# tqch/ddpm-torch

Measured on AMD Instinct MI355X. Metric: training imgs/s/GPU + 1000-step DDPM samples/s, CIFAR-10 UNet @1/2/4/8 MI355X, higher is better.
Workload: dtype bf16

## Files before the change

ddpm-torch_amd/csrc/attention.hip:

```cpp
#include "common.h"
#include "attention_common.h"
#include <string.h>

namespace {

constexpr int RB = 128;
constexpr int NT = 512;

struct AttnArgs {
    const bf16_t *q, *k, *v;  long long qkv_ld;
    const bf16_t *o, *d_o;    long long o_ld, do_ld;
    bf16_t *out;              long long out_ld;
    bf16_t *dq, *dk, *dv;     long long dqkv_ld;
    float *lse, *dvec;
    int B, L, C, Lpad;
    float scale;
};

__device__ __forceinline__ int tile_addr(int row, int col, int pitch_b, int km) {
    return row * pitch_b + ((((col >> 3) ^ (row & km))) << 4) + (col & 7) * 2;
}

template <int NJ>
struct P1 {
    f32x16 acc[2][NJ];
    __device__ __forceinline__ void zero() {
#pragma unroll
        for (int i = 0; i < 2; ++i)
#pragma unroll
            for (int j = 0; j < NJ; ++j) acc[i][j] = (f32x16)(0.f);
    }
};

__device__ __forceinline__ void wait_vm_rt(int n) {
    switch (n) {
    case 0: asm volatile("s_waitcnt vmcnt(0)" ::: "memory"); break;
    case 1: asm volatile("s_waitcnt vmcnt(1)" ::: "memory"); break;
    case 2: asm volatile("s_waitcnt vmcnt(2)" ::: "memory"); break;
    case 3: asm volatile("s_waitcnt vmcnt(3)" ::: "memory"); break;
    case 4: asm volatile("s_waitcnt vmcnt(4)" ::: "memory"); break;
    case 5: asm volatile("s_waitcnt vmcnt(5)" ::: "memory"); break;
    case 6: asm volatile("s_waitcnt vmcnt(6)" ::: "memory"); break;
    case 7: asm volatile("s_waitcnt vmcnt(7)" ::: "memory"); break;
    default: asm volatile("s_waitcnt vmcnt(8)" ::: "memory"); break;
    }
}

#ifdef ATTN_TIMING
__device__ unsigned long long* g_attn_timing = nullptr;
#define ATTN_STAMP(slot) do { if (g_attn_timing && threadIdx.x == 0) g_attn_timing[(blockIdx.y * gridDim.x + blockIdx.x) * 8 + (slot)] = wall_clock64(); } while (0)
#else
#define ATTN_STAMP(slot)
#endif

constexpr int P1_RING = 3, P2_RING = 5;
constexpr int P2_SLOT = 2 * NT * 16;
__device__ __host__ __forceinline__ int p1_slot_bytes(int Lpad) { return RB * 128 + ((Lpad + 63) / 64) * 8192; }
__device__ __host__ __forceinline__ int p2_rows(int C) { return C > 256 ? 16 : (C > 128 ? 32 : 64); }

template <int NJ, bool PIPE = true>
__device__ __forceinline__ void product_nt(P1<NJ>& t, const Opnd& X, int r0, const Opnd& Y, int Lpad, int C, char* lds, int tid) {
    const int lane = tid & 63, wr = (tid >> 8) & 1, wc = (tid >> 6) & 3;
    const int wave = __builtin_amdgcn_readfirstlane(tid >> 6);
    const int nyi = (Lpad + 63) / 64;
    const int xs_bytes = RB * 128, slot_bytes = p1_slot_bytes(Lpad), per = 2 + nyi;
    const unsigned lds0 = lds_addr(lds);
    const int nchunks = (C + 63) / 64;
    unsigned xo[2], yo[4]; int xc[2], yc[4];
#pragma unroll
    for (int i = 0; i < 2; ++i) {
        const int v = tid + NT * i, row = v >> 3;
        xc[i] = ((v & 7) ^ ((row >> 1) & 7)) * 8;
        xo[i] = (unsigned)(((long long)(r0 + row) * X.ld + xc[i]) * 2);
    }
#pragma unroll
    for (int i = 0; i < 4; ++i) {
        const int v = tid + NT * i, row = v >> 3;
        yc[i] = ((v & 7) ^ ((row >> 1) & 7)) * 8;
        yo[i] = row < Lpad ? (unsigned)(((long long)row * Y.ld + yc[i]) * 2) : BUF_OOB;
    }
    auto issue = [&](int ch) {
        char* slot = lds + (ch % P1_RING) * slot_bytes;
        const int c0 = ch * 64;
#pragma unroll
        for (int i = 0; i < 2; ++i) {
            unsigned o = c0 + xc[i] < C ? xo[i] + (unsigned)(c0 * 2) : BUF_OOB;
            asm volatile("" : "+v"(o));
            LDS_DMA16(X.rsrc, slot + (i * NT + wave * 64) * 16, o, 0);
        }
#pragma unroll
        for (int i = 0; i < 4; ++i) {
            if (i < nyi) {
                unsigned o = (yo[i] != BUF_OOB && c0 + yc[i] < C) ? yo[i] + (unsigned)(c0 * 2) : BUF_OOB;
                asm volatile("" : "+v"(o));
                LDS_DMA16(Y.rsrc, slot + xs_bytes + (i * NT + wave * 64) * 16, o, 0);
            }
        }
    };
    issue(0);
    if (nchunks > 1) issue(1);
    const int sw = (lane >> 5) ^ ((lane >> 1) & 7);
    const unsigned arow = (unsigned)((wr * 64 + (lane & 31)) * 128), brow = (unsigned)(xs_bytes + (wc * 32 + (lane & 31)) * 128);
    bool jok[NJ];
#pragma unroll
    for (int j = 0; j < NJ; ++j) jok[j] = (wc + 4 * j) * 32 < Lpad;
#ifdef ATTN_TIMING
    unsigned long long tq[5] = {0, 0, 0, 0, 0};
#define P1_T(k) do { if (ch == 1) tq[k] = clock64(); } while (0)
#else
#define P1_T(k)
#endif
    for (int ch = 0; ch < nchunks; ++ch) {
        P1_T(0);
        wait_vm_rt(ch + 1 < nchunks ? per : 0);
        P1_T(1);
        __builtin_amdgcn_s_barrier();
        P1_T(2);
        if (ch + 2 < nchunks) issue(ch + 2);
        P1_T(3);
        const unsigned cur = lds0 + (unsigned)((ch % P1_RING) * slot_bytes);
        constexpr int NS = PIPE ? 2 : 1;
        u32x4 fa[NS][2], fb[NS][NJ];
        auto rd = [&](int kc, int set) {
            const unsigned ko = (unsigned)(((2 * kc) ^ sw) << 4);
#pragma unroll
            for (int i = 0; i < 2; ++i) fa[set][i] = lds_rd16(cur + arow + (unsigned)(i * 32 * 128) + ko);
#pragma unroll
            for (int j = 0; j < NJ; ++j) fb[set][j] = lds_rd16(cur + (jok[j] ? brow + (unsigned)(j * 128 * 128) : (unsigned)xs_bytes) + ko);
        };
        rd(0, 0);
#pragma unroll
        for (int kc = 0; kc < 4; ++kc) {
            constexpr int cs = NS == 2 ? 1 : 0;
            if (NS == 1) { if (kc > 0) rd(kc, 0); lds_wait_n<0>(); }
            else if (kc < 3) { rd(kc + 1, (kc + 1) & 1); lds_wait_n<2 + NJ>(); } else lds_wait_n<0>();
#pragma unroll
            for (int i = 0; i < 2; ++i)
#pragma unroll
                for (int j = 0; j < NJ; ++j)
                    if (jok[j]) t.acc[i][j] = __builtin_amdgcn_mfma_f32_32x32x16_bf16(as_frag(fa[kc & cs][i]), as_frag(fb[kc & cs][j]), t.acc[i][j], 0, 0, 0);
            __builtin_amdgcn_sched_barrier(0);
        }
        P1_T(4);
    }
#ifdef ATTN_TIMING
    if (g_attn_timing && threadIdx.x == 0 && tq[4])
        g_attn_timing[(blockIdx.y * gridDim.x + blockIdx.x) * 8 + 7] = ((tq[1] - tq[0]) & 0xffff) | (((tq[2] - tq[1]) & 0xffff) << 16) | (((tq[3] - tq[2]) & 0xffff) << 32) | (((tq[4] - tq[3]) & 0xffff) << 48);
#endif
#undef P1_T
    __syncthreads();
}

template <int NJ2>
__device__ __forceinline__ void product_nn(f32x16 (&z)[2][NJ2], const char* tile, int pitch_b, int km, const Opnd& Y, int L, int Lpad, int C,
                                           char* ring, int tid) {
    const int lane = tid & 63, wr = (tid >> 8) & 1, wc = (tid >> 6) & 3;
    const int wave = __builtin_amdgcn_readfirstlane(tid >> 6);
    const int KR = p2_rows(C);
    const int row_b = C * 2, cpr = C >> 3;
    const int nvec = KR * cpr;
    const int skey = C % 128 == 0 ? 2 : 0;
#pragma unroll
    for (int i = 0; i < 2; ++i)
#pragma unroll
        for (int j = 0; j < NJ2; ++j) z[i][j] = (f32x16)(0.f);
    const int nchunks = (Lpad + KR - 1) / KR;
    int vkr[2]; unsigned vo[2];
#pragma unroll
    for (int i = 0; i < 2; ++i) {
        const int v = tid + NT * i;
        const int kr = v / cpr, pc = v - kr * cpr;
        const int lc = skey ? (pc ^ ((kr & 3) << 2)) : pc;
        vkr[i] = v < nvec ? kr : (1 << 20);
        vo[i] = (unsigned)(((long long)kr * Y.ld + lc * 8) * 2);
    }
    const unsigned kstep = (unsigned)((long long)KR * Y.ld * 2);
    auto issue = [&](int ch) {
        char* slot = ring + (ch % P2_RING) * P2_SLOT;
#pragma unroll
        for (int i = 0; i < 2; ++i) {
            unsigned o = ch * KR + vkr[i] < L ? vo[i] + (unsigned)ch * kstep : BUF_OOB;
            asm volatile("" : "+v"(o));
            LDS_DMA16(Y.rsrc, slot + (i * NT + wave * 64) * 16, o, 0);
        }
    };
    for (int c = 0; c < P2_RING - 1 && c < nchunks; ++c) issue(c);
    const int i16 = lane & 15;
    const unsigned tile0 = lds_addr(tile), ring0 = lds_addr(ring);
    bool jok[NJ2];
#pragma unroll
    for (int j = 0; j < NJ2; ++j) jok[j] = (wc + 4 * j) * 32 < C;
    for (int ch = 0; ch < nchunks; ++ch) {
        const int ahead = min(ch + P2_RING - 2, nchunks - 1) - ch;
        wait_vm_rt(2 * ahead);
        __builtin_amdgcn_s_barrier();
        if (ch + P2_RING - 1 < nchunks) issue(ch + P2_RING - 1);
        const unsigned cur = ring0 + (unsigned)((ch % P2_RING) * P2_SLOT);
        constexpr int NS = NJ2 <= 2 ? 2 : 1;
        u32x4 fa[NS][2]; uint2 fb[NS][NJ2][2];
        const int nks = min(KR / 16, (Lpad - ch * KR + 15) / 16);
        auto rd = [&](int ks, int set) {
            const int kg = ch * KR + ks * 16;
#pragma unroll
            for (int i = 0; i < 2; ++i) {
                const int row = wr * 64 + i * 32 + (lane & 31);
                fa[set][i] = lds_rd16(tile0 + (unsigned)(row * pitch_b + ((((kg >> 3) + (lane >> 5)) ^ (row & km)) << 4)));
            }
#pragma unroll
            for (int j = 0; j < NJ2; ++j) {
                const int ct = jok[j] ? wc + 4 * j : wc;
                const int mcol = ct * 32 + ((lane >> 4) & 1) * 16 + (i16 & 3) * 4;
                const int krow = ks * 16 + (lane >> 5) * 8 + (i16 >> 2);
                const int pch = skey ? ((mcol >> 3) ^ ((krow & 3) << 2)) : (mcol >> 3);
                const unsigned p = cur + (unsigned)(krow * row_b + pch * 16 + (mcol & 7) * 2);
                fb[set][j][0] = lds_rd_tr(p); fb[set][j][1] = lds_rd_tr(p + (unsigned)(4 * row_b));
            }
        };
        rd(0, 0);
        for (int ks = 0; ks < nks; ks += 2) {
#pragma unroll
            for (int h = 0; h < 2; ++h) {
                if (ks + h >= nks) break;
                constexpr int cs = NS == 2 ? 1 : 0;
                const int cur_set = h & cs;
                if (NS == 1) { if (ks + h > 0) rd(ks + h, 0); lds_wait_n<0>(); }
                else if (ks + h + 1 < nks) { rd(ks + h + 1, (h + 1) & 1); lds_wait_n<2 + 2 * NJ2>(); } else lds_wait_n<0>();
#pragma unroll
                for (int j = 0; j < NJ2; ++j) {
                    if (!jok[j]) continue;
                    u32x4 b4; b4.x = fb[cur_set][j][0].x; b4.y = fb[cur_set][j][0].y; b4.z = fb[cur_set][j][1].x; b4.w = fb[cur_set][j][1].y;
#pragma unroll
                    for (int i = 0; i < 2; ++i) z[i][j] = __builtin_amdgcn_mfma_f32_32x32x16_bf16(as_frag(fa[cur_set][i]), as_frag(b4), z[i][j], 0, 0, 0);
                }
                __builtin_amdgcn_sched_barrier(0);
            }
        }
    }
    __syncthreads();
}

template <int CNT, int OFF, typename Op>
__device__ __forceinline__ float half_reduce(const float (&v)[CNT], int lane, Op&& op) {
    if constexpr (CNT == 1) return v[0];
    else {
        const bool bit = (lane & OFF) != 0;
        float o[CNT / 2];
#pragma unroll
        for (int k = 0; k < CNT / 2; ++k) {
            const float send = bit ? v[k] : v[k + CNT / 2], keep = bit ? v[k + CNT / 2] : v[k];
            o[k] = op(keep, __shfl_xor(send, OFF, 64));
        }
        return half_reduce<CNT / 2, OFF / 2>(o, lane, op);
    }
}

__device__ __forceinline__ int acc_row(int r, int lane) { return (r & 3) + 8 * (r >> 2) + 4 * (lane >> 5); }

template <int NJ, typename F>
__device__ __forceinline__ void write_tile(const P1<NJ>& t, char* tile, int pitch_b, int km, int Lpad, int tid, F&& f) {
    const int lane = tid & 63, wave = tid >> 6, wr = wave >> 2, wc = wave & 3;
#pragma unroll
    for (int i = 0; i < 2; ++i)
#pragma unroll
        for (int j = 0; j < NJ; ++j) {
            const int ct = wc + 4 * j;
            if (ct * 32 >= Lpad) continue;
#pragma unroll
            for (int r = 0; r < 16; ++r) {
                const int row = wr * 64 + i * 32 + acc_row(r, lane), col = ct * 32 + (lane & 31);
                *reinterpret_cast<bf16_t*>(tile + tile_addr(row, col, pitch_b, km)) = f2bf(f(t.acc[i][j][r], i, j, r, row, col));
            }
        }
}

template <int NJ2>
__device__ __forceinline__ void store_rows(const f32x16 (&z)[2][NJ2], bf16_t* out, long long ld, int r0, int L, int C, int tid) {
    const int lane = tid & 63, wave = tid >> 6, wr = wave >> 2, wc = wave & 3;
#pragma unroll
    for (int i = 0; i < 2; ++i)
#pragma unroll
        for (int j = 0; j < NJ2; ++j) {
            const int ct = wc + 4 * j;
            if (ct * 32 >= C) continue;
#pragma unroll
            for (int r = 0; r < 16; ++r) {
                const int row = r0 + wr * 64 + i * 32 + acc_row(r, lane);
                if (row < L) out[(long long)row * ld + ct * 32 + (lane & 31)] = f2bf(z[i][j][r]);
            }
        }
}

__device__ __forceinline__ void attn_block(int B, int& b, int& r0) {
    const int gx = gridDim.x;
    if (gx > 1 && (B & 7) == 0) {
        const int L = blockIdx.y * gx + blockIdx.x, k = L >> 3;
        r0 = (k % gx) * RB;
        b = (k / gx) * 8 + (L & 7);
    } else { b = blockIdx.y; r0 = blockIdx.x * RB; }
}

struct Lds {
    char* tile; char* stage; float* red;
    int pitch_b, km;
};
__device__ __forceinline__ Lds carve(char* smem, int Lpad) {
    Lds l;
    l.pitch_b = Lpad * 2;
    const int nch = Lpad >> 3;
    int span = 4;
    while (span < 16 && nch % (span * 2) == 0) span *= 2;
    l.km = span - 1;
    l.tile = smem;
    l.stage = smem + RB * l.pitch_b;
    l.red = nullptr;
    return l;
}

template <int NJ1, int NJ2>
__global__ __launch_bounds__(NT, 2)
void attn_fwd_lse_kernel(AttnArgs a) {
    extern __shared__ __attribute__((aligned(16))) char smem[];
    const int tid = threadIdx.x, lane = tid & 63, wave = tid >> 6, wr = wave >> 2, wc = wave & 3;
    int b, r0;
    attn_block(a.B, b, r0);
    Lds l = carve(smem, a.Lpad);
    const Opnd Q = make_opnd(a.q + (long long)b * a.L * a.qkv_ld, a.qkv_ld, a.L, a.C);
    const Opnd K = make_opnd(a.k + (long long)b * a.L * a.qkv_ld, a.qkv_ld, a.L, a.C);
    const Opnd V = make_opnd(a.v + (long long)b * a.L * a.qkv_ld, a.qkv_ld, a.L, a.C);
    ATTN_STAMP(0);
    P1<NJ1> s;
    s.zero();
    product_nt<NJ1, (NJ2 <= 2)>(s, Q, r0, K, a.Lpad, a.C, smem, tid);
    ATTN_STAMP(1);
    float* red = reinterpret_cast<float*>(l.stage);
    const int kk = lane & 31, myrow = wr * 64 + (kk >> 4) * 32 + acc_row(kk & 15, lane);
    float vals[32];
#pragma unroll
    for (int i = 0; i < 2; ++i)
#pragma unroll
        for (int r = 0; r < 16; ++r) {
            float m = -3.0e38f;
#pragma unroll
            for (int j = 0; j < NJ1; ++j) {
                const int col = (wc + 4 * j) * 32 + (lane & 31);
                const float v = col < a.L ? s.acc[i][j][r] * a.scale : -3.0e38f;
                s.acc[i][j][r] = v;
                m = fmaxf(m, v);
            }
            vals[i * 16 + r] = m;
        }
    red[wc * RB + myrow] = half_reduce<32, 16>(vals, lane, [](float x, float y) { return fmaxf(x, y); });
    __syncthreads();
#pragma unroll
    for (int i = 0; i < 2; ++i)
#pragma unroll
        for (int r = 0; r < 16; ++r) {
            const int row = wr * 64 + i * 32 + acc_row(r, lane);
            const float m = fmaxf(fmaxf(red[row], red[RB + row]), fmaxf(red[2 * RB + row], red[3 * RB + row]));
            float sum = 0.f;
#pragma unroll
            for (int j = 0; j < NJ1; ++j) {
                const int col = (wc + 4 * j) * 32 + (lane & 31);
                const float e = col < a.L ? __expf(s.acc[i][j][r] - m) : 0.f;
                s.acc[i][j][r] = e;
                sum += e;
            }
            vals[i * 16 + r] = sum;
        }
    float* rsum = red + 4 * RB;
    rsum[wc * RB + myrow] = half_reduce<32, 16>(vals, lane, [](float x, float y) { return x + y; });
    __syncthreads();
    float rinv[2][16];
#pragma unroll
    for (int i = 0; i < 2; ++i)
#pragma unroll
        for (int r = 0; r < 16; ++r) {
            const int row = wr * 64 + i * 32 + acc_row(r, lane);
            const float tot = (rsum[row] + rsum[RB + row]) + (rsum[2 * RB + row] + rsum[3 * RB + row]);
            rinv[i][r] = __builtin_amdgcn_rcpf(tot);
        }
    if (a.lse && tid < RB && r0 + tid < a.L) {
        const float m = fmaxf(fmaxf(red[tid], red[RB + tid]), fmaxf(red[2 * RB + tid], red[3 * RB + tid]));
        const float tot = (rsum[tid] + rsum[RB + tid]) + (rsum[2 * RB + tid] + rsum[3 * RB + tid]);
        a.lse[(long long)b * a.L + r0 + tid] = m + __logf(tot);
    }
    __syncthreads();
    ATTN_STAMP(2);
    write_tile<NJ1>(s, l.tile, l.pitch_b, l.km, a.Lpad, tid, [&](float e, int i, int, int r, int, int) { return e * rinv[i][r]; });
    __syncthreads();
    ATTN_STAMP(3);
    f32x16 z[2][NJ2];
    product_nn<NJ2>(z, l.tile, l.pitch_b, l.km, V, a.L, a.Lpad, a.C, l.stage, tid);
    ATTN_STAMP(4);
    store_rows<NJ2>(z, a.out + (long long)b * a.L * a.out_ld, a.out_ld, r0, a.L, a.C, tid);
    ATTN_STAMP(5);
#ifdef ATTN_TIMING
    asm volatile("s_waitcnt vmcnt(0)" ::: "memory");
#endif
    ATTN_STAMP(6);
}

template <int NJ1, int NJ2>
__global__ __launch_bounds__(NT, 2)
void attn_bwd_dq_kernel(AttnArgs a) {
    extern __shared__ __attribute__((aligned(16))) char smem[];
    const int tid = threadIdx.x, lane = tid & 63, wave = tid >> 6, wr = wave >> 2, wc = wave & 3;
    int b, r0;
    attn_block(a.B, b, r0);
    Lds l = carve(smem, a.Lpad);
    const Opnd Q = make_opnd(a.q + (long long)b * a.L * a.qkv_ld, a.qkv_ld, a.L, a.C);
    const Opnd K = make_opnd(a.k + (long long)b * a.L * a.qkv_ld, a.qkv_ld, a.L, a.C);
    const Opnd V = make_opnd(a.v + (long long)b * a.L * a.qkv_ld, a.qkv_ld, a.L, a.C);
    const Opnd dO = make_opnd(a.d_o + (long long)b * a.L * a.do_ld, a.do_ld, a.L, a.C);
    float* dloc = reinterpret_cast<float*>(l.tile);
    {
        const int row = tid >> 2, part = tid & 3, q = r0 + row;
        float acc = 0.f;
        if (q < a.L) {
            const bf16_t* po = a.o + ((long long)b * a.L + q) * a.o_ld;
            const bf16_t* pd = a.d_o + ((long long)b * a.L + q) * a.do_ld;
            for (int c = part * 8; c < a.C; c += 32) {
                float fo[8], fd[8];
                Elem<bf16_t>::unpack(ldg16(po + c), fo); Elem<bf16_t>::unpack(ldg16(pd + c), fd);
#pragma unroll
                for (int e = 0; e < 8; ++e) acc += fo[e] * fd[e];
            }
        }
        acc += __shfl_xor(acc, 1, 64); acc += __shfl_xor(acc, 2, 64);
        if (part == 0) { dloc[row] = acc; if (q < a.L) a.dvec[(long long)b * a.L + q] = acc; }
    }
    __syncthreads();
    float drow[2][16], lrow[2][16];
#pragma unroll
    for (int i = 0; i < 2; ++i)
#pragma unroll
        for (int r = 0; r < 16; ++r) {
            const int row = wr * 64 + i * 32 + acc_row(r, lane), q = r0 + row;
            drow[i][r] = dloc[row];
            lrow[i][r] = q < a.L ? a.lse[(long long)b * a.L + q] : 0.f;
        }
    __syncthreads();
    P1<NJ1> p;
    p.zero();
    product_nt<NJ1, (NJ2 <= 2)>(p, Q, r0, K, a.Lpad, a.C, smem, tid);
#pragma unroll
    for (int i = 0; i < 2; ++i)
#pragma unroll
        for (int j = 0; j < NJ1; ++j)
#pragma unroll
            for (int r = 0; r < 16; ++r) {
                const int col = (wc + 4 * j) * 32 + (lane & 31);
                p.acc[i][j][r] = col < a.L ? __expf(p.acc[i][j][r] * a.scale - lrow[i][r]) : 0.f;
            }
    P1<NJ1> dp;
    dp.zero();
    product_nt<NJ1, (NJ2 <= 2)>(dp, dO, r0, V, a.Lpad, a.C, smem, tid);
    write_tile<NJ1>(dp, l.tile, l.pitch_b, l.km, a.Lpad, tid,
                    [&](float v, int i, int j, int r, int, int) { return p.acc[i][j][r] * (v - drow[i][r]) * a.scale; });
    __syncthreads();
    f32x16 z[2][NJ2];
    product_nn<NJ2>(z, l.tile, l.pitch_b, l.km, K, a.L, a.Lpad, a.C, l.stage, tid);
    store_rows<NJ2>(z, a.dq + (long long)b * a.L * a.dqkv_ld, a.dqkv_ld, r0, a.L, a.C, tid);
}

template <int NJ1, int NJ2>
__global__ __launch_bounds__(NT, 2)
void attn_bwd_dkv_kernel(AttnArgs a) {
    extern __shared__ __attribute__((aligned(16))) char smem[];
    const int tid = threadIdx.x, lane = tid & 63, wave = tid >> 6, wc = wave & 3;
    int b, r0;
    attn_block(a.B, b, r0);
    Lds l = carve(smem, a.Lpad);
    const Opnd Q = make_opnd(a.q + (long long)b * a.L * a.qkv_ld, a.qkv_ld, a.L, a.C);
    const Opnd K = make_opnd(a.k + (long long)b * a.L * a.qkv_ld, a.qkv_ld, a.L, a.C);
    const Opnd V = make_opnd(a.v + (long long)b * a.L * a.qkv_ld, a.qkv_ld, a.L, a.C);
    const Opnd dO = make_opnd(a.d_o + (long long)b * a.L * a.do_ld, a.do_ld, a.L, a.C);
    float lcol[NJ1], dcol[NJ1];
#pragma unroll
    for (int j = 0; j < NJ1; ++j) {
        const int q = (wc + 4 * j) * 32 + (lane & 31);
        lcol[j] = q < a.L ? a.lse[(long long)b * a.L + q] : 0.f;
        dcol[j] = q < a.L ? a.dvec[(long long)b * a.L + q] : 0.f;
    }
    P1<NJ1> p;
    p.zero();
    product_nt<NJ1, (NJ2 <= 2)>(p, K, r0, Q, a.Lpad, a.C, smem, tid);
#pragma unroll
    for (int i = 0; i < 2; ++i)
#pragma unroll
        for (int j = 0; j < NJ1; ++j)
#pragma unroll
            for (int r = 0; r < 16; ++r) {
                const int q = (wc + 4 * j) * 32 + (lane & 31);
                p.acc[i][j][r] = q < a.L ? __expf(p.acc[i][j][r] * a.scale - lcol[j]) : 0.f;
            }
    write_tile<NJ1>(p, l.tile, l.pitch_b, l.km, a.Lpad, tid, [&](float v, int, int, int, int, int) { return v; });
    __syncthreads();
    f32x16 z[2][NJ2];
    product_nn<NJ2>(z, l.tile, l.pitch_b, l.km, dO, a.L, a.Lpad, a.C, l.stage, tid);
    store_rows<NJ2>(z, a.dv + (long long)b * a.L * a.dqkv_ld, a.dqkv_ld, r0, a.L, a.C, tid);
    P1<NJ1> dp;
    dp.zero();
    product_nt<NJ1, (NJ2 <= 2)>(dp, V, r0, dO, a.Lpad, a.C, smem, tid);
    write_tile<NJ1>(dp, l.tile, l.pitch_b, l.km, a.Lpad, tid,
                    [&](float v, int i, int j, int r, int, int) { return p.acc[i][j][r] * (v - dcol[j]) * a.scale; });
    __syncthreads();
    product_nn<NJ2>(z, l.tile, l.pitch_b, l.km, Q, a.L, a.Lpad, a.C, l.stage, tid);
    store_rows<NJ2>(z, a.dk + (long long)b * a.L * a.dqkv_ld, a.dqkv_ld, r0, a.L, a.C, tid);
}

static int check_common(const void* qkv, long long ld, int B, int L, int C, int dtype) {
    if (!qkv) return DDPM_ERR_NULL;
    if (dtype != DDPM_BF16) return DDPM_ERR_DTYPE;
    if (B <= 0 || L <= 0 || L > 256 || L % 16 || C <= 0 || C > 512 || C % 32 || ld < 3 * C) return DDPM_ERR_SHAPE;
    if (!aligned16(qkv) || ld % 8) return DDPM_ERR_ALIGN;
    if ((long long)L * ld * 2 > BUF_OOB) return DDPM_ERR_SHAPE;
    return DDPM_OK;
}

static size_t lds_bytes(int Lpad, int C) {
    const size_t tile = (size_t)RB * Lpad * 2;
    const int nch1 = (C + 63) / 64, nch2 = (Lpad + p2_rows(C) - 1) / p2_rows(C);
    const size_t p1 = (size_t)(nch1 < P1_RING ? nch1 : P1_RING) * p1_slot_bytes(Lpad);
    size_t p2 = (size_t)(nch2 < P2_RING ? nch2 : P2_RING) * P2_SLOT;
    const size_t red = 8 * RB * sizeof(float);
    if (p2 < red) p2 = red;
    return p1 > tile + p2 ? p1 : tile + p2;
}

#define ATTN_DISPATCH(KERNEL, grid, lds, st, a)                                                                            \
    do {                                                                                                                   \
        const int nj1 = (a.Lpad / 32 + 3) / 4, nj2 = (a.C / 32 + 3) / 4;                                                   \
        auto go = [&](auto k) -> int {                                                                                     \
            if (hipFuncSetAttribute(reinterpret_cast<const void*>(k), hipFuncAttributeMaxDynamicSharedMemorySize, 160 * 1024) != hipSuccess) return DDPM_ERR_LAUNCH; \
            hipLaunchKernelGGL(k, grid, dim3(NT), lds, st, a);                                                             \
            return check_launch();                                                                                         \
        };                                                                                                                 \
        if (nj1 <= 1 && nj2 <= 1) return go(&KERNEL<1, 1>);                                                                \
        if (nj1 <= 1 && nj2 <= 2) return go(&KERNEL<1, 2>);                                                                \
        if (nj1 <= 1) return go(&KERNEL<1, 4>);                                                                            \
        if (nj2 <= 1) return go(&KERNEL<2, 1>);                                                                            \
        if (nj2 <= 2) return go(&KERNEL<2, 2>);                                                                            \
        return go(&KERNEL<2, 4>);                                                                                          \
    } while (0)

}

#ifdef ATTN_TIMING
extern "C" int ddpm_debug_set_attn_timing(void* p) { return hipMemcpyToSymbol(HIP_SYMBOL(g_attn_timing), &p, sizeof(p)) == hipSuccess ? 0 : -1; }
#endif

extern "C" int ddpm_attention_fwd_lse(const void* qkv, long long ld, void* out, long long out_ld, float* lse, int B, int L, int C, float scale,
                                      int dtype, void* stream) {
    int rc = check_common(qkv, ld, B, L, C, dtype);
    if (rc) return rc;
    if (!out) return DDPM_ERR_NULL;
    if (!aligned16(out) || out_ld % 8) return DDPM_ERR_ALIGN;
    AttnArgs a; memset(&a, 0, sizeof(a));
    a.q = (const bf16_t*)qkv; a.k = a.q + C; a.v = a.q + 2 * C; a.qkv_ld = ld;
    a.out = (bf16_t*)out; a.out_ld = out_ld; a.lse = lse;
    a.B = B; a.L = L; a.C = C; a.Lpad = (L + 31) / 32 * 32; a.scale = scale;
    const dim3 grid((L + RB - 1) / RB, B);
    const size_t lds = lds_bytes(a.Lpad, C);
    hipStream_t st = (hipStream_t)stream;
    ATTN_DISPATCH(attn_fwd_lse_kernel, grid, lds, st, a);
}

extern "C" int ddpm_attention_bwd(const void* qkv, long long ld, const void* o, long long o_ld, const void* d_o, long long do_ld,
                                  const float* lse, float* dvec, void* dqkv, long long dqkv_ld, int B, int L, int C, float scale,
                                  int dtype, void* stream) {
    int rc = check_common(qkv, ld, B, L, C, dtype);
    if (rc) return rc;
    if (!o || !d_o || !lse || !dvec || !dqkv) return DDPM_ERR_NULL;
    if (!aligned16(o) || !aligned16(d_o) || !aligned16(dqkv) || o_ld % 8 || do_ld % 8 || dqkv_ld % 8 || dqkv_ld < 3 * C) return DDPM_ERR_ALIGN;
    if (do_ld < C || (long long)L * do_ld * 2 > BUF_OOB) return DDPM_ERR_SHAPE;
    AttnArgs a; memset(&a, 0, sizeof(a));
    a.q = (const bf16_t*)qkv; a.k = a.q + C; a.v = a.q + 2 * C; a.qkv_ld = ld;
    a.o = (const bf16_t*)o; a.o_ld = o_ld; a.d_o = (const bf16_t*)d_o; a.do_ld = do_ld;
    a.dq = (bf16_t*)dqkv; a.dk = a.dq + C; a.dv = a.dq + 2 * C; a.dqkv_ld = dqkv_ld;
    a.lse = const_cast<float*>(lse); a.dvec = dvec;
    a.B = B; a.L = L; a.C = C; a.Lpad = (L + 31) / 32 * 32; a.scale = scale;
    const dim3 grid((L + RB - 1) / RB, B);
    const size_t lds = lds_bytes(a.Lpad, C);
    hipStream_t st = (hipStream_t)stream;
    {
        auto run = [&]() -> int { ATTN_DISPATCH(attn_bwd_dq_kernel, grid, lds, st, a); };
        rc = run();
        if (rc) return rc;
    }
    ATTN_DISPATCH(attn_bwd_dkv_kernel, grid, lds, st, a);
}
```

Baseline: 14790.

## Hand off dS from dK/dV kernel to a lightweight dQ kernel

When Lpad <= C, the dK/dV backward kernel now runs first. It computes the row sums D = rowsum(O*dO) itself, with the loads overlapped with the first QK^T product. It also writes the bf16 dS tile, transposed, into the dQ output buffer as scratch. A new dQ kernel then loads dS straight into LDS and does only dS·K, instead of recomputing P and dP. This removes two matmuls and the exp work from the dQ pass. The cost is extra global writes and reads of an L×L scratch tile, and more register pressure in the dK/dV kernel.

```diff
diff --git a/ddpm-torch_amd/csrc/attention.hip b/ddpm-torch_amd/csrc/attention.hip
--- a/ddpm-torch_amd/csrc/attention.hip
+++ b/ddpm-torch_amd/csrc/attention.hip
@@ -58,8 +58,19 @@
 __device__ __host__ __forceinline__ int p1_slot_bytes(int Lpad) { return RB * 128 + ((Lpad + 63) / 64) * 8192; }
 __device__ __host__ __forceinline__ int p2_rows(int C) { return C > 256 ? 16 : (C > 128 ? 32 : 64); }
 
-template <int NJ, bool PIPE = true>
-__device__ __forceinline__ void product_nt(P1<NJ>& t, const Opnd& X, int r0, const Opnd& Y, int Lpad, int C, char* lds, int tid) {
+__device__ __host__ __forceinline__ size_t lds_bytes(int Lpad, int C) {
+    const size_t tile = (size_t)RB * Lpad * 2;
+    const int nch1 = (C + 63) / 64, nch2 = (Lpad + p2_rows(C) - 1) / p2_rows(C);
+    const size_t p1 = (size_t)(nch1 < P1_RING ? nch1 : P1_RING) * p1_slot_bytes(Lpad);
+    size_t p2 = (size_t)(nch2 < P2_RING ? nch2 : P2_RING) * P2_SLOT;
+    const size_t red = 8 * RB * sizeof(float);
+    if (p2 < red) p2 = red;
+    return p1 > tile + p2 ? p1 : tile + p2;
+}
+
+struct NoPre { __device__ __forceinline__ void operator()() const {} };
+template <int NJ, bool PIPE = true, typename Pre = NoPre>
+__device__ __forceinline__ void product_nt(P1<NJ>& t, const Opnd& X, int r0, const Opnd& Y, int Lpad, int C, char* lds, int tid, const Pre& pre = Pre()) {
     const int lane = tid & 63, wr = (tid >> 8) & 1, wc = (tid >> 6) & 3;
     const int wave = __builtin_amdgcn_readfirstlane(tid >> 6);
     const int nyi = (Lpad + 63) / 64;
@@ -99,6 +110,7 @@
     };
     issue(0);
     if (nchunks > 1) issue(1);
+    pre();
     const int sw = (lane >> 5) ^ ((lane >> 1) & 7);
     const unsigned arow = (unsigned)((wr * 64 + (lane & 31)) * 128), brow = (unsigned)(xs_bytes + (wc * 32 + (lane & 31)) * 128);
     bool jok[NJ];
@@ -269,6 +281,34 @@
             for (int r = 0; r < 16; ++r) {
                 const int row = wr * 64 + i * 32 + acc_row(r, lane), col = ct * 32 + (lane & 31);
                 *reinterpret_cast<bf16_t*>(tile + tile_addr(row, col, pitch_b, km)) = f2bf(f(t.acc[i][j][r], i, j, r, row, col));
+            }
+        }
+}
+
+template <int NJ, typename F>
+__device__ __forceinline__ void write_tile_handoff(const P1<NJ>& t, char* tile, int pitch_b, int km, int Lpad, int tid, bf16_t* dq, long long ld,
+                                                   int r0, int L, F&& f) {
+    const int lane = tid & 63, wave = tid >> 6, wr = wave >> 2, wc = wave & 3;
+#pragma unroll
+    for (int i = 0; i < 2; ++i)
+#pragma unroll
+        for (int j = 0; j < NJ; ++j) {
+            const int ct = wc + 4 * j;
+            if (ct * 32 >= Lpad) continue;
+            const int col = ct * 32 + (lane & 31);
+            bf16_t* qrow = dq + (long long)col * ld + r0;
+#pragma unroll
+            for (int g = 0; g < 4; ++g) {
+                const int row0 = wr * 64 + i * 32 + acc_row(4 * g, lane);
+                float v[4];
+#pragma unroll
+                for (int e = 0; e < 4; ++e) v[e] = f(t.acc[i][j][4 * g + e], i, j, 4 * g + e, row0 + e, col);
+                uint2 w;
+                w.x = pack_bf2(v[0], v[1]); w.y = pack_bf2(v[2], v[3]);
+                const bf16_t h[4] = {(bf16_t)(w.x & 0xffffu), (bf16_t)(w.x >> 16), (bf16_t)(w.y & 0xffffu), (bf16_t)(w.y >> 16)};
+#pragma unroll
+                for (int e = 0; e < 4; ++e) *reinterpret_cast<bf16_t*>(tile + tile_addr(row0 + e, col, pitch_b, km)) = h[e];
+                if (col < L && r0 + row0 < L) *reinterpret_cast<uint2*>(qrow + row0) = w;
             }
         }
 }
@@ -463,10 +503,8 @@
     store_rows<NJ2>(z, a.dq + (long long)b * a.L * a.dqkv_ld, a.dqkv_ld, r0, a.L, a.C, tid);
 }
 
-template <int NJ1, int NJ2>
-__global__ __launch_bounds__(NT, 2)
-void attn_bwd_dkv_kernel(AttnArgs a) {
-    extern __shared__ __attribute__((aligned(16))) char smem[];
+template <int NJ1, int NJ2, bool HANDOFF>
+__device__ __forceinline__ void attn_bwd_dkv_body(const AttnArgs& a, char* smem) {
     const int tid = threadIdx.x, lane = tid & 63, wave = tid >> 6, wc = wave & 3;
     int b, r0;
     attn_block(a.B, b, r0);
@@ -480,11 +518,58 @@
     for (int j = 0; j < NJ1; ++j) {
         const int q = (wc + 4 * j) * 32 + (lane & 31);
         lcol[j] = q < a.L ? a.lse[(long long)b * a.L + q] : 0.f;
-        dcol[j] = q < a.L ? a.dvec[(long long)b * a.L + q] : 0.f;
+        if (!HANDOFF) dcol[j] = q < a.L ? a.dvec[(long long)b * a.L + q] : 0.f;
+    }
+    float* dloc = reinterpret_cast<float*>(smem + lds_bytes(a.Lpad, a.C));
+    constexpr int G = 8;
+    const int drow = tid >> 2, dpart = tid & 3;
+    u32x4 vo[NJ1][G], vd[NJ1][G];
+    auto d_row = [&](int pass, int c0, u32x4 (&o)[G], u32x4 (&d)[G]) {
+        const long long qc = (long long)b * a.L + min(pass * RB + drow, a.L - 1);
+        const bf16_t* po = a.o + qc * a.o_ld;
+        const bf16_t* pd = a.d_o + qc * a.do_ld;
+#pragma unroll
+        for (int k = 0; k < G; ++k) {
+            const int c = min(c0 + dpart * 8 + 32 * k, a.C - 8);
+            o[k] = ldg16(po + c); d[k] = ldg16(pd + c);
+        }
+    };
+    auto d_sum = [&](float acc, int c0, const u32x4 (&o)[G], const u32x4 (&d)[G]) {
+#pragma unroll
+        for (int k = 0; k < G; ++k) {
+            float fo[8], fd[8];
+            Elem<bf16_t>::unpack(o[k], fo); Elem<bf16_t>::unpack(d[k], fd);
+            float s = acc;
+#pragma unroll
+            for (int e = 0; e < 8; ++e) s += fo[e] * fd[e];
+            acc = c0 + 32 * k < a.C ? s : acc;
+        }
+        return acc;
+    };
+    auto d_rows = [&]() {
+#pragma unroll
+        for (int pass = 0; pass < NJ1; ++pass) {
+            float acc = d_sum(0.f, 0, vo[pass], vd[pass]);
+            if constexpr (NJ2 > 2)
+                for (int c0 = 32 * G; c0 < a.C; c0 += 32 * G) {
+                    u32x4 o[G], d[G];
+                    d_row(pass, c0, o, d);
+                    acc = d_sum(acc, c0, o, d);
+                }
+            acc += __shfl_xor(acc, 1, 64); acc += __shfl_xor(acc, 2, 64);
+            const int q = pass * RB + drow;
+            if (dpart == 0 && q < a.L) { dloc[q] = acc; if (r0 == 0) a.dvec[(long long)b * a.L + q] = acc; }
+        }
+    };
+    if constexpr (HANDOFF) {
+#pragma unroll
+        for (int pass = 0; pass < NJ1; ++pass) d_row(pass, 0, vo[pass], vd[pass]);
+        __builtin_amdgcn_sched_barrier(0);
     }
     P1<NJ1> p;
     p.zero();
-    product_nt<NJ1, (NJ2 <= 2)>(p, K, r0, Q, a.Lpad, a.C, smem, tid);
+    if constexpr (HANDOFF) product_nt<NJ1, (NJ2 <= 2)>(p, K, r0, Q, a.Lpad, a.C, smem, tid, d_rows);
+    else product_nt<NJ1, (NJ2 <= 2)>(p, K, r0, Q, a.Lpad, a.C, smem, tid);
 #pragma unroll
     for (int i = 0; i < 2; ++i)
 #pragma unroll
@@ -502,11 +587,57 @@
     P1<NJ1> dp;
     dp.zero();
     product_nt<NJ1, (NJ2 <= 2)>(dp, V, r0, dO, a.Lpad, a.C, smem, tid);
-    write_tile<NJ1>(dp, l.tile, l.pitch_b, l.km, a.Lpad, tid,
-                    [&](float v, int i, int j, int r, int, int) { return p.acc[i][j][r] * (v - dcol[j]) * a.scale; });
+    auto ds = [&](float v, int i, int j, int r, int, int) { return p.acc[i][j][r] * (v - dcol[j]) * a.scale; };
+    if constexpr (HANDOFF) {
+#pragma unroll
+        for (int j = 0; j < NJ1; ++j) {
+            const int q = (wc + 4 * j) * 32 + (lane & 31);
+            dcol[j] = q < a.L ? dloc[q] : 0.f;
+        }
+        write_tile_handoff<NJ1>(dp, l.tile, l.pitch_b, l.km, a.Lpad, tid, a.dq + (long long)b * a.L * a.dqkv_ld, a.dqkv_ld, r0, a.L, ds);
+    } else {
+        write_tile<NJ1>(dp, l.tile, l.pitch_b, l.km, a.Lpad, tid, ds);
+    }
     __syncthreads();
     product_nn<NJ2>(z, l.tile, l.pitch_b, l.km, Q, a.L, a.Lpad, a.C, l.stage, tid);
     store_rows<NJ2>(z, a.dk + (long long)b * a.L * a.dqkv_ld, a.dqkv_ld, r0, a.L, a.C, tid);
+}
+
+template <int NJ1, int NJ2>
+__global__ __launch_bounds__(NT, 2)
+void attn_bwd_dkv_kernel(AttnArgs a) {
+    extern __shared__ __attribute__((aligned(16))) char smem[];
+    attn_bwd_dkv_body<NJ1, NJ2, true>(a, smem);
+}
+template <int NJ1, int NJ2>
+__global__ __launch_bounds__(NT, 2)
+void attn_bwd_dkv_dvec_kernel(AttnArgs a) {
+    extern __shared__ __attribute__((aligned(16))) char smem[];
+    attn_bwd_dkv_body<NJ1, NJ2, false>(a, smem);
+}
+
+template <int NJ2>
+__global__ __launch_bounds__(NT, 2)
+void attn_bwd_dq_ds_kernel(AttnArgs a) {
+    extern __shared__ __attribute__((aligned(16))) char smem[];
+    const int tid = threadIdx.x;
+    const int wave = __builtin_amdgcn_readfirstlane(tid >> 6);
+    int b, r0;
+    attn_block(a.B, b, r0);
+    Lds l = carve(smem, a.Lpad);
+    const Opnd K = make_opnd(a.k + (long long)b * a.L * a.qkv_ld, a.qkv_ld, a.L, a.C);
+    bf16_t* dq = a.dq + (long long)b * a.L * a.dqkv_ld;
+    const Opnd dS = make_opnd(dq, a.dqkv_ld, a.L, a.L);
+    const int cpr = a.Lpad >> 3, nti = a.Lpad >> 5;
+    for (int i = 0; i < nti; ++i) {
+        const int v = tid + NT * i, row = v / cpr, lc = (v - row * cpr) ^ (row & l.km);
+        unsigned o = (r0 + row < a.L && lc * 8 < a.L) ? (unsigned)(((long long)(r0 + row) * a.dqkv_ld + lc * 8) * 2) : BUF_OOB;
+        asm volatile("" : "+v"(o));
+        LDS_DMA16(dS.rsrc, l.tile + (i * NT + wave * 64) * 16, o, 0);
+    }
+    f32x16 z[2][NJ2];
+    product_nn<NJ2>(z, l.tile, l.pitch_b, l.km, K, a.L, a.Lpad, a.C, l.stage, tid);
+    store_rows<NJ2>(z, dq, a.dqkv_ld, r0, a.L, a.C, tid);
 }
 
 static int check_common(const void* qkv, long long ld, int B, int L, int C, int dtype) {
@@ -518,15 +649,11 @@
     return DDPM_OK;
 }
 
-static size_t lds_bytes(int Lpad, int C) {
-    const size_t tile = (size_t)RB * Lpad * 2;
-    const int nch1 = (C + 63) / 64, nch2 = (Lpad + p2_rows(C) - 1) / p2_rows(C);
-    const size_t p1 = (size_t)(nch1 < P1_RING ? nch1 : P1_RING) * p1_slot_bytes(Lpad);
-    size_t p2 = (size_t)(nch2 < P2_RING ? nch2 : P2_RING) * P2_SLOT;
-    const size_t red = 8 * RB * sizeof(float);
-    if (p2 < red) p2 = red;
-    return p1 > tile + p2 ? p1 : tile + p2;
-}
+static size_t lds_bytes_p2(int Lpad, int C) {
+    const int nch2 = (Lpad + p2_rows(C) - 1) / p2_rows(C);
+    return (size_t)RB * Lpad * 2 + (size_t)(nch2 < P2_RING ? nch2 : P2_RING) * P2_SLOT;
+}
+constexpr size_t D_BYTES = 256 * sizeof(float);
 
 #define ATTN_DISPATCH(KERNEL, grid, lds, st, a)                                                                            \
     do {                                                                                                                   \
@@ -583,10 +710,23 @@
     const dim3 grid((L + RB - 1) / RB, B);
     const size_t lds = lds_bytes(a.Lpad, C);
     hipStream_t st = (hipStream_t)stream;
+    if (a.Lpad <= C && (long long)L * dqkv_ld * 2 <= BUF_OOB) {
+        const size_t lds_dkv = lds + D_BYTES, lds_dq = lds_bytes_p2(a.Lpad, C);
+        auto dkv = [&]() -> int { ATTN_DISPATCH(attn_bwd_dkv_kernel, grid, lds_dkv, st, a); };
+        rc = dkv();
+        if (rc) return rc;
+        auto go = [&](auto k) -> int {
+            if (hipFuncSetAttribute(reinterpret_cast<const void*>(k), hipFuncAttributeMaxDynamicSharedMemorySize, 160 * 1024) != hipSuccess) return DDPM_ERR_LAUNCH;
+            hipLaunchKernelGGL(k, grid, dim3(NT), lds_dq, st, a);
+            return check_launch();
+        };
+        const int nj2 = (C / 32 + 3) / 4;
+        return nj2 <= 1 ? go(&attn_bwd_dq_ds_kernel<1>) : nj2 <= 2 ? go(&attn_bwd_dq_ds_kernel<2>) : go(&attn_bwd_dq_ds_kernel<4>);
+    }
     {
         auto run = [&]() -> int { ATTN_DISPATCH(attn_bwd_dq_kernel, grid, lds, st, a); };
         rc = run();
         if (rc) return rc;
     }
-    ATTN_DISPATCH(attn_bwd_dkv_kernel, grid, lds, st, a);
-}
+    ATTN_DISPATCH(attn_bwd_dkv_dvec_kernel, grid, lds, st, a);
+}
```

Result: no change. 14730 (-0.4%).
